# rag9704/SKIRT

Hardware: AMD Instinct MI355X
Metric: photon packets/sec (whole node), 128^3 octree, 1/2/4/8 MI355X + HBM% (higher is better)
Workload: dtype f64

## Files before the change

skirt_amd/csrc/device/engine.hip:

```cpp
#include <hip/hip_runtime.h>

#include <algorithm>
#include <cfloat>
#include <cmath>
#include <cstring>
#include <string>
#include <type_traits>
#include <vector>

#include "vor_terms.hpp"
#include "cyl2d_walk.hpp"
#include "sph_walk.hpp"
#include "geom_sample.hpp"
#include "../../../include/skirt_mcrt.h"
#include "philox.hpp"

using skirt_dev::PacketRng;

namespace {

constexpr double kDblMax = 1.7976931348623157e308;
constexpr int kBlock = 256;
constexpr int kSegWords = 3 * (kBlock / 64) * 4 / 8;
#ifndef SKIRT_LABS_BUF
// ... 55 lines not shown

struct PathRec {
    double s0, ds, tau0, dtau;
    int m, pad;
};
constexpr int kPathCap = 2048;
constexpr int kContSlots = 1 << 15;
enum ErrorBits : unsigned { ERR_TAU = 1u, ERR_PATH_CAP = 2u, ERR_QUEUE = 4u, ERR_GEOM = 8u };
static_assert(GEOMS_SHELL == SKIRT_GEOM_SHELL && GEOMS_GAMMA == SKIRT_GEOM_GAMMA && GEOMS_GAUSSIAN == SKIRT_GEOM_GAUSSIAN &&
                  GEOMS_TTAURIDISK == SKIRT_GEOM_TTAURIDISK && GEOMS_TORUS == SKIRT_GEOM_TORUS &&
                  GEOMS_CONICALSHELL == SKIRT_GEOM_CONICALSHELL,
              "geom_sample.hpp follows the kinds of skirt_mcrt.h");
template <int GRID>
constexpr bool kEnterInEvent = GRID == SKIRT_GRID_VORONOI;
constexpr int kCellIndexGroup = 2;
constexpr int kNoCell = -2;
constexpr int kOutsideShift = 28;
constexpr int kCellMaskOut = (1 << kOutsideShift) - 1;
template <int GRID>
constexpr int kSegsPerStep = GRID == SKIRT_GRID_VORONOI ? 2 : 1;

struct __attribute__((aligned(16))) DetRec {
    double Lp;
    double tau;
    int l;
    unsigned flags;
};
static_assert(sizeof(DetRec) == 24 || sizeof(DetRec) == 32, "detection record layout");
__device__ __forceinline__ unsigned rayMode(unsigned f) { return f & 3u; }
__device__ __forceinline__ unsigned rayCat(unsigned f) { return (f >> 2) & 3u; }
__device__ __forceinline__ int rayInstr(unsigned f) { return (int)((f >> 4) & 63u); }
__device__ __forceinline__ int rayLevel(unsigned f) { return (int)((f >> 10) & 255u); }
__device__ __forceinline__ int rayEll(unsigned f) { return (int)(f >> 18); }

struct LeafEntry;

struct alignas(16) BlockSite {
    double x, y, z;
    int id, pad;
};
static_assert(sizeof(BlockSite) == 32, "block site layout");

struct alignas(16) VorEntry {
    float ox, oy, oz;
    int next;
};
constexpr int kVorHead = 3;

__device__ __forceinline__ VorEntry vorEntry(const VorEntry* B, int q) {
    const float* P = reinterpret_cast<const float*>(B + kVorHead + (q & ~1));
    const int h = q & 1;
    return VorEntry{P[h], P[2 + h], P[4 + h], __float_as_int(P[6 + h])};
}

template <int N>
__device__ __forceinline__ void vorEntries(const VorEntry* B, int q0, VorEntry (&e)[N]) {
#pragma unroll
    for (int p = 0; p < N / 2; p++) {
        const float4 x = *reinterpret_cast<const float4*>(B + kVorHead + q0 + 2 * p);
        const int4 y = *reinterpret_cast<const int4*>(B + kVorHead + q0 + 2 * p + 1);
        e[2 * p] = VorEntry{x.x, x.z, __int_as_float(y.x), y.z};
        e[2 * p + 1] = VorEntry{x.y, x.w, __int_as_float(y.y), y.w};
    }
}
constexpr double kCarryTau = 0.5;
#ifndef SKIRT_POLY_EXPM1
// ... 68 lines not shown
    const double* cellCdf;
    const int* cellGuide;
    const double* cellLtot;
    double cellBias;
    const int* cellNode;
    int phase, peel;
    int ninstr;
    const DevInstr* instr;
    int nsed;
    unsigned long long npp, first, end, seed;
    unsigned long long sliceLo, sliceCnt;
    unsigned int tag;
    double minWeightReduction;
    int minScatt;
    double xi;
    int store, hasDust;
    double* labs;
    unsigned labsBytes;
    int labsGlobal;
    int labsHi;
    int labsCopies;
    unsigned labsCopyStride;
    double* tally;
    unsigned int* error;
    unsigned long long* stats;
    unsigned long long* crossed;
    int crossedBins;
    int nslots;
    double *srx, *sry, *srz, *skx, *sky, *skz, *sL, *sLth;
    int *sell, *snscatt, *sstellar, *sstate;
    int* svcell;
    uint32_t *splo, *sphi, *sblock, *sw2, *sw3, *shave;
    double *resA, *resB;
    RayRec* rays;
    DetRec* det;
    int* act[2];
    unsigned long long* claim;
    unsigned int* ctr;
    int parity, init, threshold;
    int walkBack;
    int continuous, rayCap;
    PathRec* pathBuf;
    int* pathCnt;
    int ldsMeshOff, ldsOptOff, ldsInstrOff, ldsSedOff;
    int detCopies;
};

struct __attribute__((aligned(16))) LeafEntry {
    int node;
    unsigned cl;
    double rho0;
};
constexpr int kLeafLevelShift = 27;
constexpr unsigned kLeafCellMask = (1u << kLeafLevelShift) - 1u;
constexpr int kMaxMapLevel = 9;
constexpr int kBinCellBits = 23;
constexpr unsigned kBinCellMask = (1u << kBinCellBits) - 1u;
constexpr int kMaxBinMapLevel = 7;

__host__ __device__ __forceinline__ unsigned leafBricks(int N) { return (unsigned)((N + 1) >> 1); }
__host__ __device__ __forceinline__ unsigned leafIndex(int N, unsigned x, unsigned y, unsigned z) {
    const unsigned nb = leafBricks(N);
    return ((((x >> 1) * nb + (y >> 1)) * nb + (z >> 1)) << 3) | ((x & 1u) << 2) | ((y & 1u) << 1) | (z & 1u);
}
__host__ __device__ __forceinline__ unsigned long long leafMapSize(int N) {
    const unsigned long long nb = leafBricks(N);
// ... 1012 lines not shown
            const double dx = x - sx, dy = y - sy, dz = z - sz;
            return dx * dx + dy * dy + dz * dz;
        };
        const int start = a.vorStart[m];
        double sx, sy, sz;
        siteAt(a, start, sx, sy, sz);
        const double target = d2(sx, sy, sz);
        const int cnt = reinterpret_cast<const int4*>(a.vorSlots + start + 2)->y;
        for (int q = 0; q < cnt; q++) {
            const int nxt = vorEntry(a.vorSlots + start, q).next;
            if (nxt < 0) continue;
            siteAt(a, nxt, sx, sy, sz);
            if (d2(sx, sy, sz) < target) return false;
        }
        return true;
    }
};

template <int GRID, bool ONECOMP, bool CONT, bool STORE, bool GLOBAL = false>
struct Tracer {
    const Args& a;
    const Shared& sh;
    unsigned int nseg = 0;
    unsigned int absorbs = 0, laneSlots = 0, requests = 0;
    unsigned* waveSegs;
    double* pendVal;
    unsigned* pendIdx;
    unsigned char* pendHi;
    __amdgpu_buffer_rsrc_t labsRsrc;
    unsigned copyOff = 0;
    unsigned labsOob = 0;
    int npend = 0;
    unsigned gstep = 0;

    __device__ __forceinline__ void drain() {
        static_assert(kLabsBuf >= 2 && kLabsBuf <= 64 && (kLabsBuf & (kLabsBuf - 1)) == 0, "kLabsBuf: power of 2");
        constexpr int G = 64 / kLabsBuf;
        const int lane = threadIdx.x & 63;
        const int wbase = threadIdx.x - lane;
        const int j = lane & (kLabsBuf - 1);
#pragma unroll
        for (int i = 0; i < kLabsBuf; i++) issue(i);
        npend = 0;
    }

    __device__ __forceinline__ void issue(int i) {
        constexpr int G = 64 / kLabsBuf;
        const int lane = threadIdx.x & 63;
        const int wbase = threadIdx.x - lane;
        const int j = lane & (kLabsBuf - 1);
        const int src = G * i + lane / kLabsBuf;
        const int n = __shfl(npend, src);
        const int q = j * kBlock + wbase + src;
        const unsigned idx = pendIdx[q];
        const size_t eidx = a.labsHi ? ((size_t)pendHi[q] << 32 | idx) : (size_t)idx;
        const unsigned line = (unsigned)(reinterpret_cast<size_t>(a.labs + eidx) >> 6);
        const unsigned prev = __shfl(line, lane - 1);
        const unsigned long long starts = __ballot(j < n && (j == 0 || prev != line));
        absorbs += (unsigned)__popcll(__ballot(j < n));
        requests += (unsigned)__popcll(starts);
        if constexpr (GLOBAL) {
            if (j < n) atomicAddF64(a.labs + eidx, pendVal[q]);
        } else {
            const double v = j < n ? pendVal[q] : 0.0;
            bufferAtomicAddF64(v, labsRsrc, (int)(j < n ? idx * 8u + copyOff : labsOob), 0, 0);
        }
// ... 48 lines not shown
                if (ONECOMP) albedo = sh.alb[r.ell];
                else {
                    double ksca = 0.0, kext = 0.0;
                    for (int h = 0; h < a.ncomp; h++) {
                        ksca += rho(m, h) * sh.ksca[h * a.nlambda + r.ell];
                        kext += rho(m, h) * sh.kext[h * a.nlambda + r.ell];
                    }
                    albedo = (kext > 0.0) ? ksca / kext : 0.0;
                    r.f2 += albedo * Lintm;
                }
#ifdef SKIRT_DEBUG_FILL
                printf("E S %d %.17g %.17g %.17g\n", m, ds, dtau, (1.0 - albedo) * Lintm);
#endif
                if (STORE && a.store) {
                    pendVal[npend * kBlock + threadIdx.x] = (1.0 - albedo) * Lintm;
                    if (a.labsHi) {
                        const unsigned long long e = (unsigned long long)r.ell * (unsigned)a.labsStride + (unsigned)m;
                        pendIdx[npend * kBlock + threadIdx.x] = (unsigned)e;
                        pendHi[npend * kBlock + threadIdx.x] = (unsigned char)(e >> 32);
                    } else {
                        pendIdx[npend * kBlock + threadIdx.x] = (unsigned)r.ell * (unsigned)a.labsStride + (unsigned)m;
                    }
                    npend++;
                }
            }
        } else if (r.mode == RAY_WALK) {
            if (r.tau > r.param) return false;
            r.f1 = r.tau;
            r.f2 = r.s;
        }
        return true;
    }

    __device__ __forceinline__ void load(Ray& r, unsigned id) {
        const double2* c = reinterpret_cast<const double2*>(a.rays + id);
        const double2 c0 = c[0], c1 = c[1], c2 = c[2], c3 = c[3];
        const int4 c6 = reinterpret_cast<const int4*>(c)[4];
        r.id = id;
        r.x = c0.x; r.y = c0.y; r.z = c1.x;
        r.dx = c1.y; r.dy = c2.x; r.dz = c2.y;
        r.ix = (fabs(r.dx) > 1e-15) ? 1.0 / r.dx : 0.0;
        r.iy = (fabs(r.dy) > 1e-15) ? 1.0 / r.dy : 0.0;
        r.iz = (fabs(r.dz) > 1e-15) ? 1.0 / r.dz : 0.0;
        r.param = c3.y;
        r.idx = c6.x;
        r.flags = (unsigned)c6.y;
        r.mode = rayMode(r.flags);
        r.ell = rayEll(r.flags);
        r.tau = 0;
        if (CONT && r.mode == RAY_FILL) a.pathCnt[r.idx] = 0;
#ifdef SKIRT_DEBUG_FILL
        if (r.mode == RAY_FILL)
            printf("E L %d %.17g %.17g %.17g %.17g %.17g %.17g %.17g\n", r.ell, r.x, r.y, r.z, r.dx, r.dy, r.dz, r.param);
#endif
        r.s = c3.x;
        r.kext = sh.kext[r.ell];
        r.f1 = (r.mode == RAY_FILL) ? 1.0 : 0.0;
        r.f2 = (r.mode == RAY_WALK) ? c3.x : 0.0;
        nseg = kEnterInEvent<GRID> ? ((unsigned)c6.z >> kOutsideShift) : 0u;
        if (kEnterInEvent<GRID>) {
            r.ci = c6.z & kCellMaskOut;
            r.cj = c6.w;
            r.ck = 0;
        } else if (r.mode != RAY_NONE &&
            !Grid<GRID>::begin(a, sh, r, [&](int m, double rho0, double ds) { return segment(r, m, rho0, ds); })) {
            finish(r);
            r.mode = RAY_NONE;
        }
    }

    __device__ __forceinline__ void finish(const Ray& r) {
        atomicAdd(&waveSegs[(threadIdx.x >> 6) * 3 + (r.mode == RAY_FILL ? 0 : r.mode == RAY_WALK ? 1 : 2)], nseg);
        if (a.crossed && r.mode != RAY_WALK) crossedAdd(a, nseg);
        if (r.mode == RAY_PEEL) {
            a.det[r.idx].tau = r.tau;
        } else if (r.mode == RAY_FILL) {
            a.resA[r.idx] = r.tau;
            if (!ONECOMP) a.resB[r.idx] = r.f2;
        } else {
            const double tauint = r.param;
            double s = 0;
            if (tauint > 0) {
                if (r.tau > tauint) s = r.f2 + ((tauint - r.f1) / (r.tau - r.f1)) * (r.s - r.f2);
                else s = r.f2;
            }
            a.resA[r.idx] = s;
        }
    }
};

__device__ __forceinline__ bool detectSlot(const DevInstr& ins, unsigned flags, int slot, double Lp, double Lextf,
                                           double& v) {
    v = Lextf;
    if (ins.kind != SKIRT_INSTR_FULL) return slot == 0;
    switch (rayCat(flags)) {
    case CAT_STAR_DIRECT:
        if (slot == 0) v = Lp;
        return slot <= 1;
    case CAT_STAR_SCATTERED: {
        const int lev = rayLevel(flags);
        return slot == 2 || (lev >= 1 && lev <= ins.levels && slot == 5 + lev - 1);
    }
    case CAT_DUST_DIRECT: return slot == 3;
    default: return slot == 4;
    }
}

__device__ __forceinline__ double* frameAt(const Args& a, const DevInstr& ins, int ell, int l, int slot) {
    return a.tally + ins.frameBase + ((long long)ell * ins.nx * ins.ny + l) * ins.slotStride + slot;
}

__device__ __forceinline__ void detectPeel(const Args& a, const DevInstr& ins, unsigned flags, int l, double Lp,
                                           double tau, double* sed) {
    const double Lextf = Lp * exp(-tau);
    const int nl = a.nlambda;
    const int ell = rayEll(flags);
    for (int slot = 0; slot < ins.nslots; slot++) {
        double v;
        if (!detectSlot(ins, flags, slot, Lp, Lextf, v)) continue;
        if (ins.kind != SKIRT_INSTR_FRAME) {
// ... 244 lines not shown
}

template <int GRID, bool ONECOMP, bool CONT, bool STORE, bool GLOBAL = false>
__device__ __forceinline__ void traceBody(const Args& a) {
    extern __shared__ __attribute__((aligned(16))) double lds[];
    if (blockIdx.x == 0 && threadIdx.x == 0) {
        CTR(a.ctr, 1 - a.parity) = 0;
        CTR(a.ctr, 2 + a.parity) = 0;
        CTR(a.ctr, 8 + (1 - a.parity)) = 0;
    }
    const unsigned int nfront = CTR(a.ctr, a.parity);
    if (nfront + CTR(a.ctr, 8 + a.parity) == 0) return;
    if ((unsigned long long)nfront + CTR(a.ctr, 8 + a.parity) > (unsigned long long)a.rayCap) {
        if (blockIdx.x == 0 && threadIdx.x == 0) atomicOr(a.error, ERR_QUEUE);
        return;
    }
    Shared sh = stageTables(a, lds, gridParts<GRID>() | STAGE_OPTICS);

    Tracer<GRID, ONECOMP, CONT, STORE, GLOBAL> T{a, sh};
    T.labsOob = a.labsCopies > 1 ? (unsigned)a.labsCopies * a.labsCopyStride : a.labsBytes;
    T.labsRsrc = __builtin_amdgcn_make_buffer_rsrc(a.labs, 0, (int)T.labsOob, 0x00020000);
    if (a.labsCopies > 1)
        T.copyOff = (unsigned)((blockIdx.x * (kBlock / 64) + (threadIdx.x >> 6)) % (unsigned)a.labsCopies) * a.labsCopyStride;
    T.waveSegs = reinterpret_cast<unsigned*>(lds + a.ldsInstrOff);
    T.pendVal = lds + a.ldsInstrOff + kSegWords;
    T.pendIdx = reinterpret_cast<unsigned*>(T.pendVal + kLabsBuf * kBlock);
    T.pendHi = reinterpret_cast<unsigned char*>(T.pendIdx + kLabsBuf * kBlock);
    if (threadIdx.x < 3 * (kBlock / 64)) T.waveSegs[threadIdx.x] = 0;
    __syncthreads();
    const int lane = threadIdx.x & 63;
    const unsigned int nrays = nfront + CTR(a.ctr, 8 + a.parity);
    Ray r;
    r.mode = RAY_NONE;
    bool done = false;
    constexpr unsigned kPullChunk = GRID == SKIRT_GRID_VORONOI ? 64 : 128;
    unsigned cur = 0, curEnd = 0, nxt = 0;
    bool haveNext = false;
    auto reserve = [&]() {
        unsigned int base = 0;
        if (lane == 0) base = atomicAdd(CTRP(a.ctr, 4), kPullChunk);
        return __shfl(base, 0);
    };
    while (true) {
        const bool idle = (r.mode == RAY_NONE) && !done;
        const unsigned long long imask = __ballot(idle);
        const unsigned long long amask = __ballot(r.mode != RAY_NONE);
        if (imask == 0 && amask == 0) break;
        if (imask != 0 && (amask == 0 || __popcll(imask) >= a.threshold)) {
            const unsigned int rank = (unsigned int)__popcll(imask & ((1ull << lane) - 1ull));
            const unsigned int k = (unsigned int)__popcll(imask);
            const unsigned int avail = curEnd - cur;
            if (avail < k && !haveNext) { nxt = reserve(); haveNext = true; }
            const unsigned int id = rank < avail ? cur + rank : nxt + (rank - avail);
            if (avail >= k) cur += k;
            else { cur = nxt + (k - avail); curEnd = nxt + kPullChunk; haveNext = false; }
            if (!haveNext && curEnd - cur < kPullChunk / 2 && cur < nrays) { nxt = reserve(); haveNext = true; }
            if (idle) {
                if (id >= nrays) done = true;
                else T.load(r, id < nfront ? id : (unsigned)a.rayCap - 1u - (id - nfront));
            }
            __builtin_amdgcn_s_waitcnt(0x0F70);
        }
#pragma unroll 1
        for (int it = 0; it < kStepsPerPull; it++) {
            const unsigned long long live = __ballot(r.mode != RAY_NONE);
            if (live == 0) break;
            T.laneSlots += 64;
            auto seg = [&](int m, double rho0, double ds) { return T.segment(r, m, rho0, ds); };
            if (r.mode != RAY_NONE) {
                if (!Grid<GRID>::step(a, sh, r, seg)) {
                    T.finish(r);
                    r.mode = RAY_NONE;
                }
            }
            if constexpr (!STORE) {
            } else if constexpr (kSegsPerStep<GRID> == 1) {
                T.drainStep();
            } else if (SKIRT_VOR_DRAIN2) {
                static_assert(kSegsPerStep<GRID> == 2, "two drains per step hold two adds per step");
                T.drainStep2();
            } else {
                if (__ballot(T.npend > kLabsBuf - kSegsPerStep<GRID>)) T.drain();
            }
        }
    }
    if constexpr (STORE) T.drain();
    const unsigned* ws = T.waveSegs + (threadIdx.x >> 6) * 3;
    const bool l0 = lane == 0;
    const unsigned long long vals[8] = {0, l0 ? ws[0] : 0u, l0 ? ws[1] : 0u, l0 ? ws[2] : 0u, 0,
                                        l0 ? T.absorbs : 0u, l0 ? T.laneSlots : 0u, l0 ? T.requests : 0u};
    flushStats(a, vals);
}
// ... 43 lines not shown
            }
            if (l >= 0 && ins.kind != SKIRT_INSTR_SED) atomicAddF64(frameAt(a, ins, ell, l, slot), v);
        }
        if (sub == 0) detects++;
    }
    __syncthreads();
    for (int q = threadIdx.x; copies && q < a.nsed; q += blockDim.x) {
        double v = 0.0;
        for (int g = 0; g < copies; g++) v += sh.sed[g * a.nsed + q];
        if (v != 0.0) {
            int ii = 0;
            while (ii + 1 < a.ninstr && sh.instr[ii + 1].sedOff <= q) ii++;
            atomicAddF64(a.tally + sh.instr[ii].sedBase + (q - sh.instr[ii].sedOff), v);
        }
    }
    const unsigned long long vals[8] = {0, 0, 0, 0, detects, 0, 0, 0};
    flushStats(a, vals);
}

struct Packet {
    double rx, ry, rz, kx, ky, kz, L, Lth;
    int ell, nscatt, stellar, state;
    PacketRng rng;
};

template <int GRID, bool ONECOMP>
struct Events {
    const Args& a;
    const Shared& sh;
    unsigned int packets = 0, detects = 0, segFill = 0, segWalk = 0, segPeel = 0;

    __device__ __forceinline__ double rho(int m, int h) const { return a.rho[(size_t)m * a.ncomp + h]; }

    __device__ __forceinline__ void emitRay(unsigned pos, const Packet& p, double dx, double dy, double dz, double prm,
                                            int idx, unsigned flags, int& vcell) {
        Ray r;
        r.x = p.rx; r.y = p.ry; r.z = p.rz;
        r.dx = dx; r.dy = dy; r.dz = dz;
        r.ix = (fabs(dx) > 1e-15) ? 1.0 / dx : 0.0;
        r.iy = (fabs(dy) > 1e-15) ? 1.0 / dy : 0.0;
        r.iz = (fabs(dz) > 1e-15) ? 1.0 / dz : 0.0;
        r.s = 0;
        r.ci = r.cj = 0;
        const unsigned mode = rayMode(flags);
        int4* dst = reinterpret_cast<int4*>(a.rays + pos);
        bool entered = a.hasDust;
        unsigned nseg = 0;
        if constexpr (kEnterInEvent<GRID>) {
            if (entered) entered = Grid<GRID>::beginAt(a, r, vcell, [&](int, double, double ds) {
                if (ds > 0) { r.s += ds; nseg++; }
                return true;
            });
        }
        if (kEnterInEvent<GRID> && a.crossed && mode != RAY_WALK && a.hasDust) {
            if (!entered) crossedAdd(a, 0);
        }
        if (!entered) {
            if (mode != RAY_PEEL) {
                a.resA[idx] = 0.0;
                if (!ONECOMP) a.resB[idx] = 0.0;
                if (mode == RAY_FILL && a.continuous) a.pathCnt[idx] = 0;
            }
            dst[4] = make_int4(idx, (int)RAY_NONE, 0, 0);
            return;
        }
        double2* d2 = reinterpret_cast<double2*>(dst);
        d2[0] = make_double2(r.x, r.y);
        d2[1] = make_double2(r.z, dx);
        d2[2] = make_double2(dy, dz);
        d2[3] = make_double2(r.s, prm);
        dst[4] = make_int4(idx, (int)flags, r.ci | (int)(min(nseg, 7u) << kOutsideShift), r.cj);
    }

    __device__ __forceinline__ void load(int s, Packet& p) const {
        p.rx = a.srx[s]; p.ry = a.sry[s]; p.rz = a.srz[s];
        p.kx = a.skx[s]; p.ky = a.sky[s]; p.kz = a.skz[s];
        p.L = a.sL[s]; p.Lth = a.sLth[s];
        p.ell = a.sell[s]; p.nscatt = a.snscatt[s]; p.stellar = a.sstellar[s]; p.state = a.sstate[s];
        p.rng.k0 = (uint32_t)a.seed; p.rng.k1 = (uint32_t)(a.seed >> 32); p.rng.tag = a.tag;
        p.rng.plo = a.splo[s]; p.rng.phi = a.sphi[s]; p.rng.block = a.sblock[s];
        p.rng.w2 = a.sw2[s]; p.rng.w3 = a.sw3[s]; p.rng.have = a.shave[s];
    }
    __device__ __forceinline__ void store(int s, const Packet& p) const {
        a.srx[s] = p.rx; a.sry[s] = p.ry; a.srz[s] = p.rz;
        a.skx[s] = p.kx; a.sky[s] = p.ky; a.skz[s] = p.kz;
        a.sL[s] = p.L; a.sLth[s] = p.Lth;
        a.sell[s] = p.ell; a.snscatt[s] = p.nscatt; a.sstellar[s] = p.stellar; a.sstate[s] = p.state;
        a.splo[s] = p.rng.plo; a.sphi[s] = p.rng.phi; a.sblock[s] = p.rng.block;
        a.sw2[s] = p.rng.w2; a.sw3[s] = p.rng.w3; a.shave[s] = p.rng.have;
    }

    __device__ __forceinline__ int pixel(const DevInstr& ins, const Packet& p) const {
        const double xpp = -ins.sinphi * p.rx + ins.cosphi * p.ry;
        const double ypp = -ins.cosphi * ins.costheta * p.rx - ins.sinphi * ins.costheta * p.ry + ins.sintheta * p.rz;
        const double xp = ins.cospa * xpp - ins.sinpa * ypp;
        const double yp = ins.sinpa * xpp + ins.cospa * ypp;
        const int i = static_cast<int>(floor((xp - ins.xpmin) / ins.xpsiz));
        const int j = static_cast<int>(floor((yp - ins.ypmin) / ins.ypsiz));
        return (i < 0 || i >= ins.nx || j < 0 || j >= ins.ny) ? -1 : i + ins.nx * j;
    }

    __device__ __forceinline__ bool peelWeight(const DevInstr& ins, const Packet& p, double kx, double ky, double kz,
                                               double& I) const {
        const double cosalpha = kx * ins.kobs[0] + ky * ins.kobs[1] + kz * ins.kobs[2];
// ... 276 lines not shown
        p.ell = ell;
        int h = 0;
        double L = L0;
        const int N = a.nstar;
        if (N > 1) {
            const double X = p.rng.uniform();
            const double xi = a.emissionBias;
            if (X < xi) h = max(0, min(N - 1, static_cast<int>(N * X / xi)));
            else {
                const double* Xv = a.cdf + (size_t)ell * (N + 1);
                const double q = (X - xi) / (1.0 - xi);
                if (!(q < Xv[0])) {
                    int lo = -1, hi = N;
                    while (hi - lo > 1) { const int jm = (hi + lo) >> 1; if (q < Xv[jm]) hi = jm; else lo = jm; }
                    h = lo;
                }
            }
            const double Lh = a.lum[(size_t)h * a.nlambda + ell];
            if (!(Lh > 0)) return false;
            const double Lmean = a.lumtot[ell] / N;
            L = L0 * (1.0 / (1.0 - xi + xi * Lmean / Lh));
        }
        if (!launchPosition(a.geomParam + 8 * h, a.geomTable, h, p.rng, p.rx, p.ry, p.rz)) {
            atomicOr(a.error, ERR_GEOM);
            return false;
        }
        isotropic(p.rng, p.kx, p.ky, p.kz);
        p.L = L;
        p.nscatt = 0;
        p.stellar = h;
        return true;
    }

    __device__ __forceinline__ double sampleTau(Packet& p, double taupath) const {
        double tauint = -1.0;
        if (a.xi != 0.0) {
            const double X = p.rng.uniform();
            if (X < a.xi) tauint = p.rng.uniform() * taupath;
        }
        if (tauint < 0.0) {
            if (taupath < 1e-10) tauint = p.rng.uniform() * taupath;
            else {
                const double norm = 1.0 - exp(-taupath);
                double x = -log(1.0 - p.rng.uniform() * norm);
                while (x > taupath) x = -log(1.0 - p.rng.uniform() * norm);
                tauint = x;
            }
        }
        if (a.xi != 0.0) {
            const double pr = -exp(-tauint) / expm1(-taupath);
            const double q = (1.0 - a.xi) * pr + a.xi / taupath;
            p.L = p.L * (pr / q);
        }
        return tauint;
    }
};

enum PeelKind : int { PEEL_NONE = 0, PEEL_EMISSION = 1, PEEL_SCATTER = 2 };

template <class T0, class T1>
__device__ __forceinline__ void blockReserve(T0* ctr0, T0 c0, T0& r0, T1* ctr1, T1 c1, T1& r1, unsigned long long* scratch) {
    const int lane = threadIdx.x & 63, wave = threadIdx.x >> 6;
    constexpr int W = kBlock / 64;
    T0 i0 = c0;
    T1 i1 = c1;
#pragma unroll
    for (int off = 1; off < 64; off <<= 1) {
        const T0 v0 = __shfl_up(i0, off);
        const T1 v1 = __shfl_up(i1, off);
        if (lane >= off) { i0 += v0; i1 += v1; }
    }
    if (lane == 63) { scratch[wave] = (unsigned long long)i0; scratch[W + wave] = (unsigned long long)i1; }
    __syncthreads();
    T0 w0 = 0, t0 = 0;
    T1 w1 = 0, t1 = 0;
#pragma unroll
    for (int w = 0; w < W; w++) {
        const T0 s0 = (T0)scratch[w];
        const T1 s1 = (T1)scratch[W + w];
        if (w < wave) { w0 += s0; w1 += s1; }
        t0 += s0; t1 += s1;
    }
    if (threadIdx.x == 0) scratch[2 * W] = (ctr0 && t0) ? (unsigned long long)atomicAdd(ctr0, t0) : 0ull;
    if (threadIdx.x == 64) scratch[2 * W + 1] = (ctr1 && t1) ? (unsigned long long)atomicAdd(ctr1, t1) : 0ull;
    __syncthreads();
    r0 = (T0)scratch[2 * W] + w0 + i0 - c0;
    r1 = (T1)scratch[2 * W + 1] + w1 + i1 - c1;
// ... 73 lines not shown
}

__device__ __forceinline__ unsigned long long globalPacket(const Args& a, unsigned long long j) {
    if (a.sliceCnt == a.npp) return j;
    const unsigned long long ell = j / a.sliceCnt;
    return ell * a.npp + a.sliceLo + (j - ell * a.sliceCnt);
}

template <int GRID, bool ONECOMP>
__global__ void __launch_bounds__(kBlock) SKIRT_EVENT_ATTR eventKernel(const Args a) {
    __shared__ unsigned long long resv[4 * (kBlock / 64) + 4];
    extern __shared__ __attribute__((aligned(16))) double lds[];
    if (blockIdx.x == 0 && threadIdx.x == 0) CTR(a.ctr, 4) = 0;
    if (!a.init && CTR(a.ctr, 2 + a.parity) == 0) return;
    Shared sh = stageTables(a, lds, gridParts<GRID>() | STAGE_OPTICS | STAGE_INSTR);
    Events<GRID, ONECOMP> E{a, sh};
    const int lane = threadIdx.x & 63;
    const unsigned long long total = a.end - a.first;
    const unsigned int nwork = a.init ? (unsigned)a.nslots : CTR(a.ctr, 2 + a.parity);
    const int* actIn = a.act[a.parity];
    int* actOut = a.act[1 - a.parity];
    const unsigned int stride = gridDim.x * blockDim.x;
    const unsigned int rounds = (nwork + stride - 1) / stride;
    const unsigned int w0 = blockIdx.x * blockDim.x + threadIdx.x;
    int slotNext = (w0 < nwork) ? (a.init ? (int)w0 : actIn[w0]) : 0;
    for (unsigned int round = 0; round < rounds; round++) {
        const unsigned int w = round * stride + w0;
        const bool valid = w < nwork;
        const int slot = slotNext;
        const unsigned int wn = w + stride;
        if (round + 1 < rounds) slotNext = (wn < nwork) ? (a.init ? (int)wn : actIn[wn]) : 0;
        Packet p;
        p.state = S_NEW;
        double resA = 0.0, resB = 0.0;
        int vcell = kNoCell;
        if (valid && !a.init) {
            E.load(slot, p);
            resA = a.resA[slot];
            if (!ONECOMP) resB = a.resB[slot];
            if (kEnterInEvent<GRID>) vcell = a.svcell[slot];
        }
        int peel = PEEL_NONE;
        unsigned mainMode = RAY_NONE;
        double mainParam = 0;
        double ox = 0, oy = 0, oz = 0;
        if (valid && !a.init) {
            if (p.state == S_FILL) {
                const double taupath = resA;
                if (taupath < 0.0 || isnan(taupath) || isinf(taupath)) {
                    atomicOr(a.error, ERR_TAU);
                    p.state = S_NEW;
                } else {
                    if (ONECOMP) p.L = p.L * sh.alb[p.ell] * (-expm1(-taupath));
                    else p.L = resB;
                    if (p.L <= 0 || (p.L <= p.Lth && p.nscatt >= a.minScatt)) {
                        p.state = S_NEW;
                    } else {
                        p.state = S_WALK;
                        double tauint = 0.0;
                        if (taupath != 0.0) tauint = E.sampleTau(p, taupath);
                        if (tauint > 0) { mainMode = RAY_WALK; mainParam = tauint; }
                        else resA = 0.0;
                    }
                }
            }
            if (p.state == S_WALK && mainMode == RAY_NONE) {
                const double s = resA;
                vcell = kNoCell;
                p.rx = p.rx + s * p.kx;
                p.ry = p.ry + s * p.ky;
                p.rz = p.rz + s * p.kz;
                bool ok = a.ninstr > 0 && a.peel && !a.continuous;
                if (ok && !ONECOMP) { double I; ok = E.peelWeight(sh.instr[0], p, p.kx, p.ky, p.kz, I); }
                if (ok) { peel = PEEL_SCATTER; ox = p.kx; oy = p.ky; oz = p.kz; }
                E.scatter(p);
                mainMode = RAY_FILL;
                mainParam = p.L;
                p.state = S_FILL;
            }
        }
        bool need = valid && p.state == S_NEW && mainMode == RAY_NONE;
        while (__syncthreads_or(need)) {
            unsigned long long idx = 0;
            unsigned int unused = 0;
            blockReserve<unsigned long long, unsigned int>(a.claim, need ? 1ull : 0ull, idx, nullptr, 0u, unused, resv);
            if (need) {
                if (idx >= total) need = false;
                else if (E.launch(p, globalPacket(a, a.first + idx))) {
                    vcell = kNoCell;
                    if (!(p.L > 0) && !a.crossed) {
                    } else if (a.hasDust) {
                        peel = (a.ninstr > 0 && a.peel) ? PEEL_EMISSION : PEEL_NONE;
                        mainMode = RAY_FILL;
                        mainParam = p.L;
                        p.state = S_FILL;
                        need = false;
// ... 6 lines not shown
                        }
                    }
                }
            }
        }
        int nray = 0;
        if (peel != PEEL_NONE) {
            for (int i = 0; i < a.ninstr; i++) {
                const DevInstr& ins = sh.instr[i];
                if (ins.kind == SKIRT_INSTR_FRAME && E.pixel(ins, p) < 0) continue;
                nray++;
            }
        }
        if (mainMode != RAY_NONE) nray++;
        const bool active = mainMode != RAY_NONE;
        const int npeel = nray - (mainMode != RAY_NONE ? 1 : 0);
        const bool back = a.walkBack && mainMode == RAY_WALK;
        unsigned int pos, apos, dpos, wpos;
        {
            unsigned* const ctrs[4] = {CTRP(a.ctr, a.parity), CTRP(a.ctr, 2 + (1 - a.parity)), CTRP(a.ctr, 5 + a.parity),
                                       CTRP(a.ctr, 8 + a.parity)};
            const unsigned cnt[4] = {(unsigned)nray - (back ? 1u : 0u), active ? 1u : 0u, (unsigned)npeel, back ? 1u : 0u};
            unsigned res[4];
            blockReserve4(ctrs, cnt, res, resv);
            pos = res[0]; apos = res[1]; dpos = res[2]; wpos = res[3];
        }
        if ((unsigned long long)pos + (unsigned)(nray - (back ? 1 : 0)) > (unsigned long long)a.rayCap ||
            (back && wpos >= (unsigned)a.rayCap) ||
            (unsigned long long)dpos + (unsigned)npeel > (unsigned long long)(a.rayCap - a.nslots)) {
            atomicOr(a.error, ERR_QUEUE);
            nray = 0;
        }
        int inext = 0;
        for (int k = 0; k < nray; k++) {
            double dx, dy, dz, prm;
            int idx;
            unsigned flags, at;
            if (k < npeel) {
                int i = inext, l;
                while (true) {
                    const DevInstr& ins = sh.instr[i];
                    l = ins.kind == SKIRT_INSTR_SED ? -1 : E.pixel(ins, p);
                    if (ins.kind == SKIRT_INSTR_FRAME && l < 0) { i++; continue; }
                    break;
                }
                inext = i + 1;
                const DevInstr& ins = sh.instr[i];
                double Lp = p.L;
                unsigned cat, level = 0;
                if (peel == PEEL_EMISSION) {
                    cat = p.stellar >= 0 ? CAT_STAR_DIRECT : CAT_DUST_DIRECT;
                } else {
                    double I = 0;
                    E.peelWeight(ins, p, ox, oy, oz, I);
                    Lp = p.L * I;
                    cat = p.stellar >= 0 ? CAT_STAR_SCATTERED : CAT_DUST_SCATTERED;
                    level = (unsigned)min(p.nscatt, 255);
                }
                dx = ins.kobs[0]; dy = ins.kobs[1]; dz = ins.kobs[2];
                prm = Lp;
                flags = RAY_PEEL | (cat << 2) | ((unsigned)i << 4) | (level << 10) | ((unsigned)p.ell << 18);
                idx = (int)(dpos + k);
                a.det[idx] = DetRec{Lp, 0.0, l, flags};
                at = pos++;
            } else {
                dx = p.kx; dy = p.ky; dz = p.kz;
                prm = mainParam;
                idx = slot;
                flags = mainMode | ((unsigned)p.ell << 18);
                at = back ? (unsigned)a.rayCap - 1u - wpos : pos++;
            }
            E.emitRay(at, p, dx, dy, dz, prm, idx, flags, vcell);
        }
        if (active) actOut[apos] = slot;
        if (valid) E.store(slot, p);
        if (kEnterInEvent<GRID> && valid) a.svcell[slot] = vcell;
    }
    const unsigned long long vals[8] = {E.packets, E.segFill, E.segWalk, E.segPeel, E.detects, 0, 0, 0};
    flushStats(a, vals);
}

template <int GRID, bool ONECOMP>
__global__ void __launch_bounds__(kBlock) contKernel(const Args a) {
    __shared__ unsigned long long resv[3 * (kBlock / 64) + 3];
    extern __shared__ __attribute__((aligned(16))) double lds[];
    const unsigned int nwork = CTR(a.ctr, 2 + a.parity);
    if (nwork == 0) return;
    Shared sh = stageTables(a, lds, gridParts<GRID>() | STAGE_OPTICS | STAGE_INSTR);
    Events<GRID, ONECOMP> E{a, sh};
    const int* actIn = a.act[a.parity];
    const unsigned int stride = gridDim.x * blockDim.x;
    const unsigned int rounds = (nwork + stride - 1) / stride;
    const int Nl = a.nlambda;
    for (unsigned int round = 0; round < rounds; round++) {
        const unsigned int w = round * stride + blockIdx.x * blockDim.x + threadIdx.x;
        const int slot = w < nwork ? actIn[w] : 0;
        Packet p;
        p.state = S_NEW;
        if (w < nwork) E.load(slot, p);
        const bool fill = w < nwork && p.state == S_FILL;
        const int nrec = fill ? a.pathCnt[slot] : 0;
        const PathRec* rec = a.pathBuf + (size_t)slot * kPathCap;
        auto weights = [&](int m, double* wv, double& albedo) {
            double ksca = 0.0, kext = 0.0;
            for (int h = 0; h < a.ncomp; h++) {
                const double rho = a.rho[(size_t)m * a.ncomp + h];
                wv[h] = rho * sh.ksca[h * Nl + p.ell];
                ksca += rho * sh.ksca[h * Nl + p.ell];
                kext += rho * sh.kext[h * Nl + p.ell];
// ... 107 lines not shown
    int* dCellGuide = nullptr;
    size_t cellGuideCount = 0;
    double cellBias = 0.5;
    int* dCellNode = nullptr;
    double* dLabsDust = nullptr;
    bool ownLabsDust = true;
    double* dLabsRep = nullptr;
    size_t labsRepBytes = 0;
    bool labsRepDirty = false;
    int emisNtemp = 0;
    double *dEmisVolume = nullptr, *dEmisKabs = nullptr, *dEmisSigma = nullptr, *dEmisMu = nullptr, *dEmisTv = nullptr,
           *dEmisPlanck = nullptr, *dEmisLambda = nullptr, *dEmisDlambda = nullptr, *dEmisScratch = nullptr;
    int* dDevCell = nullptr;
    std::vector<DevInstr> instr;
    DevInstr* dInstr = nullptr;
    size_t nInstrTally = 0;
    int nsed = 0;
    double *dLabs = nullptr, *dTally = nullptr;
    bool ownLabs = true, ownTally = true;
    unsigned long long *dClaim = nullptr, *dStats = nullptr;
    unsigned long long* dCrossed = nullptr;
    int crossedBins = 0;
    unsigned int *dError = nullptr, *dCtr = nullptr, *hCtr = nullptr;
    hipStream_t sD = nullptr;
    hipEvent_t evDetT = nullptr, evDet[2] = {}, evDetJoin = nullptr;
    std::vector<hipEvent_t> pollEv;
    int nslots = 0, rayCap = 0;
    bool poolPath = false;
    bool poolDetPair = false;
    void* dPool = nullptr;
    size_t poolBytes = 0;
    int traceGrid = 0, threshold = 0, slotsWanted = 0;
    int walkBack = getenv("SKIRT_AMD_WALK_BACK") ? atoi(getenv("SKIRT_AMD_WALK_BACK")) : -1;
    int traceBlocksPerCU = 0;
    int lastDetCopies = 0;
    double lastMs = 0;
    bool phaseTimed = false;
    std::vector<hipEvent_t> traceEv;
    int traceLaunches = 0;
    uint64_t packagesTotal = 0;
    double traceMs = 0;
    uint64_t traceLaunchesTotal = 0;
    int numCUs = 0;
    size_t ldsMax = 64 * 1024;
    int lastIterations = 0;
    SkirtReduceTallyFn reduce = nullptr;
    void* reduceUser = nullptr;
    bool instrReduced = false;
};

namespace {

int fail(SkirtMcrt* c, int code, const std::string& msg) {
    if (c) c->err = msg;
    return code;
}

#define HIPCHECK(ctx, call)                                                                    \
    do {                                                                                       \
        hipError_t e_ = (call);                                                                \
        if (e_ != hipSuccess) return fail(ctx, SKIRT_ERR_HIP, std::string(#call) + ": " + hipGetErrorString(e_)); \
    } while (0)

template <class T>
int upload(SkirtMcrt* c, T*& dst, const T* src, size_t n) {
    if (dst) { (void)hipFree(dst); dst = nullptr; }
// ... 45 lines not shown
int walkKind(const SkirtMcrt* c, bool hasDust) {
    if (c->gridKind < 0) return kOctreeNodes;
    if (c->gridKind != SKIRT_GRID_OCTREE) return c->gridKind;
    if (c->search == SKIRT_TREE_BOOKKEEPING) return kOctreeBookkeeping;
    if (c->mapL >= 0 && hasDust) return c->binTree ? kBinTreeMap : SKIRT_GRID_OCTREE;
    return kOctreeNodes;
}

const void* traceKernelOf(int kind, bool one, bool continuous, bool global, bool noStore) {
    return withWalk(kind, [&](auto g) {
        constexpr int G = decltype(g)::value;
        if constexpr (G != SKIRT_GRID_VORONOI)
            if (noStore) return (const void*)traceKernelNoStore<G>;
        return withBool(global, [&](auto gl) {
            constexpr bool L = decltype(gl)::value;
            if constexpr (G == SKIRT_GRID_VORONOI) {
                if (!continuous) return one ? (const void*)traceKernelVor<true, false, L> : (const void*)traceKernelVor<false, false, L>;
                return one ? (const void*)traceKernelVor<true, true, L> : (const void*)traceKernelVor<false, true, L>;
            } else {
                if (!continuous) return one ? (const void*)traceKernel<G, true, false, L> : (const void*)traceKernel<G, false, false, L>;
                return one ? (const void*)traceKernel<G, true, true, L> : (const void*)traceKernel<G, false, true, L>;
            }
        });
    });
}

int ensurePool(SkirtMcrt* c, int nslots, bool continuous, bool detPair) {
    const int ninstr = (int)c->instr.size();
    const size_t rays = (size_t)nslots * (1 + ninstr) + (continuous ? (size_t)nslots * kPathCap * ninstr : 0);
    if (rays >= (size_t)INT32_MAX) return fail(c, SKIRT_ERR_UNSUPPORTED, "ray queue too large");
    const int rayCap = (int)rays;
    const size_t path = continuous ? (size_t)nslots * (kPathCap * sizeof(PathRec) + sizeof(int)) : 0;
    const size_t bytes = (size_t)rayCap * sizeof(RayRec) + (detPair ? 2 : 1) * (size_t)(rayCap - nslots) * sizeof(DetRec) +
                         (size_t)nslots * (10 * 8 + 5 * 4 + 6 * 4 + 2 * 4) + path + 4096;
    if (c->dPool && c->nslots == nslots && c->rayCap == rayCap && c->poolPath == (path > 0) && c->poolDetPair == detPair)
        return SKIRT_OK;
    c->poolPath = path > 0;
    c->poolDetPair = detPair;
    if (c->dPool) { (void)hipFree(c->dPool); c->dPool = nullptr; }
    HIPCHECK(c, hipMalloc(&c->dPool, bytes));
    c->poolBytes = bytes;
    c->nslots = nslots;
    c->rayCap = rayCap;
    return SKIRT_OK;
}

void carvePool(SkirtMcrt* c, Args& a) {
    char* p = static_cast<char*>(c->dPool);
    const size_t n = (size_t)c->nslots;
    auto takeD = [&](double*& d) { d = reinterpret_cast<double*>(p); p += n * 8; };
    auto takeI = [&](int*& d) { d = reinterpret_cast<int*>(p); p += n * 4; };
    auto takeU = [&](uint32_t*& d) { d = reinterpret_cast<uint32_t*>(p); p += n * 4; };
    a.rays = reinterpret_cast<RayRec*>(p);
    p += (size_t)c->rayCap * sizeof(RayRec);
    a.det = reinterpret_cast<DetRec*>(p);
    p += (c->poolDetPair ? 2 : 1) * (size_t)(c->rayCap - c->nslots) * sizeof(DetRec);
    takeD(a.srx); takeD(a.sry); takeD(a.srz); takeD(a.skx); takeD(a.sky); takeD(a.skz); takeD(a.sL); takeD(a.sLth);
    takeD(a.resA); takeD(a.resB);
    takeI(a.sell); takeI(a.snscatt); takeI(a.sstellar); takeI(a.sstate); takeI(a.svcell);
    takeU(a.splo); takeU(a.sphi); takeU(a.sblock); takeU(a.sw2); takeU(a.sw3); takeU(a.shave);
    takeI(a.act[0]); takeI(a.act[1]);
    a.pathBuf = nullptr;
    a.pathCnt = nullptr;
    if (c->poolPath) {
        p = reinterpret_cast<char*>(((uintptr_t)p + 15) & ~(uintptr_t)15);
        a.pathBuf = reinterpret_cast<PathRec*>(p);
        p += n * kPathCap * sizeof(PathRec);
        takeI(a.pathCnt);
    }
    a.nslots = c->nslots;
    a.rayCap = c->rayCap;
    a.ctr = c->dCtr;
}

int planLeafMap(SkirtMcrt* c, const SkirtGridDesc* g) {
    c->mapL = -1;
    c->mapReady = false;
    if (c->dLeafMap) { (void)hipFree(c->dLeafMap); c->dLeafMap = nullptr; }
    const char* env = getenv("SKIRT_AMD_LEAFMAP");
    if (env && env[0] == '0') return SKIRT_OK;
    const bool bin = g->split_dir != nullptr;
    if (c->ndev >= (int)(1u << (bin ? kBinCellBits : kLeafLevelShift))) return SKIRT_OK;
    const int maxL = bin ? kMaxBinMapLevel : kMaxMapLevel;
    struct Item { int node, lv[3], idx[3]; };
    std::vector<Item> stack{{0, {0, 0, 0}, {0, 0, 0}}};
    std::vector<Item> nodes;
    nodes.reserve(g->nnodes);
    int L = 0;
    while (!stack.empty()) {
        const Item it = stack.back();
        stack.pop_back();
// ... 1096 lines not shown
    Args& a = pl.a;
    gridArgs(c, a);
    const int kind = pl.kind = walkKind(c, p->has_dust);
    if (kind == SKIRT_GRID_OCTREE || kind == kBinTreeMap) {
        if ((rc = ensureLeafMap(c))) return rc;
        a.leafMap = c->dLeafMap; a.treeT = c->dTreeT; a.mapL = c->mapL; a.mapN = c->mapN;
        a.mapInvX = c->mapInv[0]; a.mapInvY = c->mapInv[1]; a.mapInvZ = c->mapInv[2];
        a.mapX0 = c->mapOrigin[0]; a.mapY0 = c->mapOrigin[1]; a.mapZ0 = c->mapOrigin[2];
    }
    a.optics = c->dOptics;
    a.nstar = c->nstar; a.geomParam = c->dGeomParam; a.geomTable = c->dGeomTable; a.lum = c->dLum;
    a.lumtot = c->dLumtot; a.cdf = c->dCdf; a.emissionBias = c->emissionBias;
    a.ninstr = (int)c->instr.size(); a.instr = c->dInstr; a.nsed = c->nsed;
    a.npp = npp; a.first = first; a.end = first + count; a.seed = seed;
    a.sliceLo = sliceLo; a.sliceCnt = sliceCnt;
    a.tag = (unsigned)phase | (cycle << 2);
    a.phase = phase;
    a.peel = phase != SKIRT_PHASE_DUST_SELFABS;
    a.continuous = continuous ? 1 : 0;
    a.cellLv = c->dCellLv; a.cellCdf = c->dCellCdf; a.cellGuide = c->dCellGuide; a.cellLtot = c->dCellLtot; a.cellBias = c->cellBias;
    a.cellNode = c->dCellNode;
    a.minWeightReduction = p->min_weight_reduction; a.minScatt = p->min_scatt_events; a.xi = p->scatt_bias;
    a.store = phase == SKIRT_PHASE_STELLAR ? (p->store_absorption ? 1 : 0) : (phase == SKIRT_PHASE_DUST_SELFABS ? 1 : 0);
    a.hasDust = p->has_dust ? 1 : 0;
    if (a.store && !c->dLabs) return fail(c, SKIRT_ERR_STATE, "no Labs buffer");
    if ((rc = planLabs(c, phase, pl))) return rc;
    a.tally = c->dTally;
    a.error = c->dError; a.stats = c->dStats;
    a.crossed = c->dCrossed; a.crossedBins = c->crossedBins;
    a.claim = c->dClaim;
    a.threshold = c->threshold > 0 ? c->threshold : (c->gridKind == SKIRT_GRID_VORONOI ? 8 : 16);
    a.walkBack = c->walkBack >= 0 ? c->walkBack : (c->gridKind == SKIRT_GRID_VORONOI ? 1 : 0);
    if ((rc = planLds(c, pl))) return rc;
    c->lastWalk = walkOf(kind).stat;
    pl.traceFn = traceKernelOf(kind, a.ncomp == 1, continuous, a.labsGlobal != 0, pl.noStore);
    if (pl.ldsTrace > 64 * 1024)
        HIPCHECK(c, hipFuncSetAttribute(pl.traceFn, hipFuncAttributeMaxDynamicSharedMemorySize, (int)pl.ldsTrace));
    pl.tgrid = c->traceGrid;
    if (pl.tgrid <= 0) {
        int per = 0;
        if (hipOccupancyMaxActiveBlocksPerMultiprocessor(&per, pl.traceFn, kBlock, pl.ldsTrace) != hipSuccess || per < 1) per = 2;
        pl.tgrid = std::max(1, c->numCUs) * per;
        c->traceBlocksPerCU = per;
    }
#ifndef SKIRT_EVENT_BPC
#define SKIRT_EVENT_BPC 3
#endif
    const int ebpc = SKIRT_EVENT_BPC;
    pl.egrid = std::max(1, std::min((slots + kBlock - 1) / kBlock, std::max(1, c->numCUs) * ebpc));
    pl.dgrid = std::max(1, std::max(1, c->numCUs) * 4);
    return SKIRT_OK;
}

static int runIterations(SkirtMcrt* c, const PhasePlan& pl) {
    const int kind = pl.kind;
    const bool one = pl.a.ncomp == 1;
    auto launchEvent = [&](const Args& aa, hipStream_t st) {
        withWalk(kind, [&](auto g) {
            withBool(one, [&](auto o) {
                hipLaunchKernelGGL((eventKernel<decltype(g)::value, decltype(o)::value>), dim3(pl.egrid), dim3(kBlock),
                                   pl.ldsEvent, st, aa);
            });
        });
    };
    auto launchCont = [&](const Args& aa, hipStream_t st) {
        withWalk(kind, [&](auto g) {
// ... 437 lines not shown
```

Before: 237.9 million.

## Fuse fill-ray tau sampling and walk ray into the trace kernel

When a fill ray finishes in the trace kernel, the change samples the interaction optical depth in place using random draws precomputed by the event kernel, then relaunches the same ray as a walk ray within that trace pass. The goal is to avoid a separate event round and ray emission just to trace the walk, which saves a kernel round-trip and ray-record traffic. In exchange it adds per-slot buffers, more state in the ray records and Ray registers, and a fallback path when the rejection loop would need extra draws. The fused path is on by default except for Voronoi grids, continuous mode, and no-store octree-node walks.

```diff
diff --git a/skirt_amd/csrc/device/engine.hip b/skirt_amd/csrc/device/engine.hip
--- a/skirt_amd/csrc/device/engine.hip
+++ b/skirt_amd/csrc/device/engine.hip
@@ -111,6 +111,46 @@
 __device__ __forceinline__ int rayInstr(unsigned f) { return (int)((f >> 4) & 63u); }
 __device__ __forceinline__ int rayLevel(unsigned f) { return (int)((f >> 10) & 255u); }
 __device__ __forceinline__ int rayEll(unsigned f) { return (int)(f >> 18); }
+
+enum FillStatus : int { FILL_TERMINATED = 0, FILL_NO_WALK = 1, FILL_WALK = 2, FILL_FALLBACK = 3 };
+__device__ __forceinline__ double fillBiasWeight(double L, double tauint, double taupath, double xi) {
+    const double pr = -exp(-tauint) / expm1(-taupath);
+    const double q = (1.0 - xi) * pr + xi / taupath;
+    return L * (pr / q);
+}
+template <bool ONECOMP, class Draws>
+__device__ __forceinline__ int decideFill(double taupath, double& L, double Lsca, double albedo, double thr, double xi,
+                                          Draws& draws, double& tauint) {
+    tauint = 0.0;
+    if (taupath < 0.0 || isnan(taupath) || isinf(taupath)) return FILL_FALLBACK;
+    if (ONECOMP) L = L * albedo * (-expm1(-taupath));
+    else L = Lsca;
+    if (L <= 0 || L <= thr) return FILL_TERMINATED;
+    if (taupath == 0.0) return FILL_NO_WALK;
+    const bool biased = xi != 0.0 && draws.biased(xi);
+    const double u = draws.uniform();
+    double t;
+    if (biased || taupath < 1e-10) t = u * taupath;
+    else {
+        const double norm = 1.0 - exp(-taupath);
+        t = -log(1.0 - u * norm);
+        if (t > taupath) return FILL_FALLBACK;
+    }
+    if (xi != 0.0) L = fillBiasWeight(L, t, taupath, xi);
+    tauint = t;
+    return t > 0 ? FILL_WALK : FILL_NO_WALK;
+}
+struct FillDrawsStream {
+    PacketRng& rng;
+    __device__ __forceinline__ bool biased(double xi) { return rng.uniform() < xi; }
+    __device__ __forceinline__ double uniform() { return rng.uniform(); }
+};
+struct FillDrawsAhead {
+    bool b;
+    double u;
+    __device__ __forceinline__ bool biased(double) const { return b; }
+    __device__ __forceinline__ double uniform() const { return u; }
+};
 
 struct LeafEntry;
 
@@ -245,6 +285,9 @@
     int* svcell;
     uint32_t *splo, *sphi, *sblock, *sw2, *sw3, *shave;
     double *resA, *resB;
+    double* resS;
+    double *fuseU, *fuseThr;
+    int fuse;
     RayRec* rays;
     DetRec* det;
     int* act[2];
@@ -1323,6 +1366,11 @@
     unsigned labsOob = 0;
     int npend = 0;
     unsigned gstep = 0;
+    double fu = 0, fthr = 0;
+    static constexpr unsigned kLaneWalkOn = 1u << 31;
+    static constexpr bool kFuse = !CONT && (STORE || GRID != kOctreeNodes);
+    __device__ __forceinline__ double& fillThr(Ray& r) { return ONECOMP ? r.f2 : fthr; }
+    __device__ __forceinline__ double& fillU(Ray& r) { return (ONECOMP && !STORE) ? r.f1 : fu; }
 
     __device__ __forceinline__ void drain() {
         static_assert(kLabsBuf >= 2 && kLabsBuf <= 64 && (kLabsBuf & (kLabsBuf - 1)) == 0, "kLabsBuf: power of 2");
@@ -1437,7 +1485,7 @@
         return true;
     }
 
-    __device__ __forceinline__ void load(Ray& r, unsigned id) {
+    __device__ __forceinline__ void load(Ray& r, unsigned id, bool walkOn) {
         const double2* c = reinterpret_cast<const double2*>(a.rays + id);
         const double2 c0 = c[0], c1 = c[1], c2 = c[2], c3 = c[3];
         const int4 c6 = reinterpret_cast<const int4*>(c)[4];
@@ -1450,6 +1498,10 @@
         r.param = c3.y;
         r.idx = c6.x;
         r.flags = (unsigned)c6.y;
+        if (kFuse && walkOn) {
+            r.param = fillU(r);
+            r.flags = (r.flags & ~3u) | RAY_WALK;
+        }
         r.mode = rayMode(r.flags);
         r.ell = rayEll(r.flags);
         r.tau = 0;
@@ -1458,10 +1510,14 @@
         if (r.mode == RAY_FILL)
             printf("E L %d %.17g %.17g %.17g %.17g %.17g %.17g %.17g\n", r.ell, r.x, r.y, r.z, r.dx, r.dy, r.dz, r.param);
 #endif
-        r.s = c3.x;
+        r.s = kEnterInEvent<GRID> ? c3.x : 0.0;
         r.kext = sh.kext[r.ell];
         r.f1 = (r.mode == RAY_FILL) ? 1.0 : 0.0;
-        r.f2 = (r.mode == RAY_WALK) ? c3.x : 0.0;
+        r.f2 = (r.mode == RAY_WALK) ? r.s : 0.0;
+        if (kFuse && a.fuse && r.mode == RAY_FILL) {
+            fillU(r) = kEnterInEvent<GRID> ? a.fuseU[r.idx] : __hiloint2double(c6.w, c6.z);
+            fillThr(r) = kEnterInEvent<GRID> ? a.fuseThr[r.idx] : c3.x;
+        }
         nseg = kEnterInEvent<GRID> ? ((unsigned)c6.z >> kOutsideShift) : 0u;
         if (kEnterInEvent<GRID>) {
             r.ci = c6.z & kCellMaskOut;
@@ -1474,14 +1530,30 @@
         }
     }
 
-    __device__ __forceinline__ void finish(const Ray& r) {
+    __device__ __forceinline__ void finish(Ray& r) {
         atomicAdd(&waveSegs[(threadIdx.x >> 6) * 3 + (r.mode == RAY_FILL ? 0 : r.mode == RAY_WALK ? 1 : 2)], nseg);
         if (a.crossed && r.mode != RAY_WALK) crossedAdd(a, nseg);
+        unsigned walkOn = 0;
+        double* const walked = (kFuse && a.fuse) ? a.resS : a.resA;
         if (r.mode == RAY_PEEL) {
             a.det[r.idx].tau = r.tau;
         } else if (r.mode == RAY_FILL) {
             a.resA[r.idx] = r.tau;
             if (!ONECOMP) a.resB[r.idx] = r.f2;
+            if (kFuse && a.fuse) {
+                const double u = fillU(r);
+                FillDrawsAhead draws{u < 0.0, fabs(u)};
+                double L = r.param, tauint;
+                int st = decideFill<ONECOMP>(r.tau, L, r.f2, ONECOMP ? sh.alb[r.ell] : 0.0,
+                                              ONECOMP ? r.f2 : fthr, a.xi, draws, tauint);
+                if (a.fuse == 2 && (r.idx & 1)) st = FILL_FALLBACK;
+                if (st == FILL_WALK) {
+                    fillU(r) = tauint;
+                    walkOn = kLaneWalkOn | r.id;
+                } else {
+                    a.resS[r.idx] = -1.0;
+                }
+            }
         } else {
             const double tauint = r.param;
             double s = 0;
@@ -1489,8 +1561,9 @@
                 if (r.tau > tauint) s = r.f2 + ((tauint - r.f1) / (r.tau - r.f1)) * (r.s - r.f2);
                 else s = r.f2;
             }
-            a.resA[r.idx] = s;
-        }
+            walked[r.idx] = s;
+        }
+        r.id = walkOn;
     }
 };
 
@@ -1801,6 +1874,7 @@
     const unsigned int nrays = nfront + CTR(a.ctr, 8 + a.parity);
     Ray r;
     r.mode = RAY_NONE;
+    r.id = 0;
     bool done = false;
     constexpr unsigned kPullChunk = GRID == SKIRT_GRID_VORONOI ? 64 : 128;
     unsigned cur = 0, curEnd = 0, nxt = 0;
@@ -1816,8 +1890,10 @@
         const unsigned long long amask = __ballot(r.mode != RAY_NONE);
         if (imask == 0 && amask == 0) break;
         if (imask != 0 && (amask == 0 || __popcll(imask) >= a.threshold)) {
-            const unsigned int rank = (unsigned int)__popcll(imask & ((1ull << lane) - 1ull));
-            const unsigned int k = (unsigned int)__popcll(imask);
+            const bool walkOn = idle && (r.id & T.kLaneWalkOn) != 0;
+            const unsigned long long pmask = imask & ~__ballot(walkOn);
+            const unsigned int rank = (unsigned int)__popcll(pmask & ((1ull << lane) - 1ull));
+            const unsigned int k = (unsigned int)__popcll(pmask);
             const unsigned int avail = curEnd - cur;
             if (avail < k && !haveNext) { nxt = reserve(); haveNext = true; }
             const unsigned int id = rank < avail ? cur + rank : nxt + (rank - avail);
@@ -1825,8 +1901,8 @@
             else { cur = nxt + (k - avail); curEnd = nxt + kPullChunk; haveNext = false; }
             if (!haveNext && curEnd - cur < kPullChunk / 2 && cur < nrays) { nxt = reserve(); haveNext = true; }
             if (idle) {
-                if (id >= nrays) done = true;
-                else T.load(r, id < nfront ? id : (unsigned)a.rayCap - 1u - (id - nfront));
+                if (!walkOn && id >= nrays) done = true;
+                else T.load(r, walkOn ? r.id & ~T.kLaneWalkOn : id < nfront ? id : (unsigned)a.rayCap - 1u - (id - nfront), walkOn);
             }
             __builtin_amdgcn_s_waitcnt(0x0F70);
         }
@@ -1936,7 +2012,7 @@
 
     __device__ __forceinline__ double rho(int m, int h) const { return a.rho[(size_t)m * a.ncomp + h]; }
 
-    __device__ __forceinline__ void emitRay(unsigned pos, const Packet& p, double dx, double dy, double dz, double prm,
+    __device__ __forceinline__ bool emitRay(unsigned pos, const Packet& p, double dx, double dy, double dz, double prm,
                                             int idx, unsigned flags, int& vcell) {
         Ray r;
         r.x = p.rx; r.y = p.ry; r.z = p.rz;
@@ -1962,11 +2038,12 @@
         if (!entered) {
             if (mode != RAY_PEEL) {
                 a.resA[idx] = 0.0;
+                if (mode == RAY_WALK && a.fuse) a.resS[idx] = 0.0;
                 if (!ONECOMP) a.resB[idx] = 0.0;
                 if (mode == RAY_FILL && a.continuous) a.pathCnt[idx] = 0;
             }
             dst[4] = make_int4(idx, (int)RAY_NONE, 0, 0);
-            return;
+            return false;
         }
         double2* d2 = reinterpret_cast<double2*>(dst);
         d2[0] = make_double2(r.x, r.y);
@@ -1974,6 +2051,7 @@
         d2[2] = make_double2(dy, dz);
         d2[3] = make_double2(r.s, prm);
         dst[4] = make_int4(idx, (int)flags, r.ci | (int)(min(nseg, 7u) << kOutsideShift), r.cj);
+        return true;
     }
 
     __device__ __forceinline__ void load(int s, Packet& p) const {
@@ -2316,27 +2394,14 @@
         return true;
     }
 
-    __device__ __forceinline__ double sampleTau(Packet& p, double taupath) const {
-        double tauint = -1.0;
-        if (a.xi != 0.0) {
-            const double X = p.rng.uniform();
-            if (X < a.xi) tauint = p.rng.uniform() * taupath;
-        }
-        if (tauint < 0.0) {
-            if (taupath < 1e-10) tauint = p.rng.uniform() * taupath;
-            else {
-                const double norm = 1.0 - exp(-taupath);
-                double x = -log(1.0 - p.rng.uniform() * norm);
-                while (x > taupath) x = -log(1.0 - p.rng.uniform() * norm);
-                tauint = x;
-            }
-        }
-        if (a.xi != 0.0) {
-            const double pr = -exp(-tauint) / expm1(-taupath);
-            const double q = (1.0 - a.xi) * pr + a.xi / taupath;
-            p.L = p.L * (pr / q);
-        }
-        return tauint;
+    __device__ __forceinline__ double fillThreshold(const Packet& p) const { return p.nscatt >= a.minScatt ? p.Lth : 0.0; }
+
+    __device__ __forceinline__ double exponCutoffAgain(Packet& p, double taupath) const {
+        const double norm = 1.0 - exp(-taupath);
+        double x = -log(1.0 - p.rng.uniform() * norm);
+        while (x > taupath) x = -log(1.0 - p.rng.uniform() * norm);
+        if (a.xi != 0.0) p.L = fillBiasWeight(p.L, x, taupath, a.xi);
+        return x;
     }
 };
 
@@ -2476,12 +2541,16 @@
         if (round + 1 < rounds) slotNext = (wn < nwork) ? (a.init ? (int)wn : actIn[wn]) : 0;
         Packet p;
         p.state = S_NEW;
-        double resA = 0.0, resB = 0.0;
+        double resA = 0.0, resB = 0.0, resS = -1.0;
         int vcell = kNoCell;
         if (valid && !a.init) {
             E.load(slot, p);
             resA = a.resA[slot];
             if (!ONECOMP) resB = a.resB[slot];
+            if (a.fuse) {
+                resS = a.resS[slot];
+                if (p.state == S_WALK) resA = resS;
+            }
             if (kEnterInEvent<GRID>) vcell = a.svcell[slot];
         }
         int peel = PEEL_NONE;
@@ -2491,21 +2560,27 @@
         if (valid && !a.init) {
             if (p.state == S_FILL) {
                 const double taupath = resA;
-                if (taupath < 0.0 || isnan(taupath) || isinf(taupath)) {
-                    atomicOr(a.error, ERR_TAU);
+                FillDrawsStream draws{p.rng};
+                double tauint;
+                int st = decideFill<ONECOMP>(taupath, p.L, resB, ONECOMP ? sh.alb[p.ell] : 0.0, E.fillThreshold(p), a.xi,
+                                             draws, tauint);
+                if (st == FILL_FALLBACK) {
+                    if (taupath < 0.0 || isnan(taupath) || isinf(taupath)) {
+                        atomicOr(a.error, ERR_TAU);
+                        st = FILL_TERMINATED;
+                    } else {
+                        tauint = E.exponCutoffAgain(p, taupath);
+                        st = tauint > 0 ? FILL_WALK : FILL_NO_WALK;
+                    }
+                    resS = -1.0;
+                }
+                if (st == FILL_TERMINATED) {
                     p.state = S_NEW;
                 } else {
-                    if (ONECOMP) p.L = p.L * sh.alb[p.ell] * (-expm1(-taupath));
-                    else p.L = resB;
-                    if (p.L <= 0 || (p.L <= p.Lth && p.nscatt >= a.minScatt)) {
-                        p.state = S_NEW;
-                    } else {
-                        p.state = S_WALK;
-                        double tauint = 0.0;
-                        if (taupath != 0.0) tauint = E.sampleTau(p, taupath);
-                        if (tauint > 0) { mainMode = RAY_WALK; mainParam = tauint; }
-                        else resA = 0.0;
-                    }
+                    p.state = S_WALK;
+                    if (st == FILL_WALK && resS >= 0.0) resA = resS;
+                    else if (st == FILL_WALK) { mainMode = RAY_WALK; mainParam = tauint; }
+                    else resA = 0.0;
                 }
             }
             if (p.state == S_WALK && mainMode == RAY_NONE) {
@@ -2578,6 +2653,7 @@
             nray = 0;
         }
         int inext = 0;
+        int fillAt = -1;
         for (int k = 0; k < nray; k++) {
             double dx, dy, dz, prm;
             int idx;
@@ -2616,11 +2692,27 @@
                 flags = mainMode | ((unsigned)p.ell << 18);
                 at = back ? (unsigned)a.rayCap - 1u - wpos : pos++;
             }
-            E.emitRay(at, p, dx, dy, dz, prm, idx, flags, vcell);
+            const bool in = E.emitRay(at, p, dx, dy, dz, prm, idx, flags, vcell);
+            if (k >= npeel && in && mainMode == RAY_FILL) fillAt = (int)at;
         }
         if (active) actOut[apos] = slot;
         if (valid) E.store(slot, p);
         if (kEnterInEvent<GRID> && valid) a.svcell[slot] = vcell;
+        if (a.fuse && fillAt >= 0) {
+            PacketRng ahead = p.rng;
+            const bool biased = a.xi != 0.0 && ahead.uniform() < a.xi;
+            const double u = ahead.uniform();
+            const double fu = biased ? -u : u, fthr = E.fillThreshold(p);
+            RayRec* rec = a.rays + fillAt;
+            if (kEnterInEvent<GRID>) {
+                a.fuseU[slot] = fu;
+                a.fuseThr[slot] = fthr;
+            } else {
+                rec->s0 = fthr;
+                rec->ci = __double2loint(fu);
+                rec->cj = __double2hiint(fu);
+            }
+        }
     }
     const unsigned long long vals[8] = {E.packets, E.segFill, E.segWalk, E.segPeel, E.detects, 0, 0, 0};
     flushStats(a, vals);
@@ -2794,6 +2886,7 @@
     size_t poolBytes = 0;
     int traceGrid = 0, threshold = 0, slotsWanted = 0;
     int walkBack = getenv("SKIRT_AMD_WALK_BACK") ? atoi(getenv("SKIRT_AMD_WALK_BACK")) : -1;
+    int fuseWalk = getenv("SKIRT_AMD_FUSE_WALK") ? atoi(getenv("SKIRT_AMD_FUSE_WALK")) : -1;
     int traceBlocksPerCU = 0;
     int lastDetCopies = 0;
     double lastMs = 0;
@@ -2905,7 +2998,7 @@
     const int rayCap = (int)rays;
     const size_t path = continuous ? (size_t)nslots * (kPathCap * sizeof(PathRec) + sizeof(int)) : 0;
     const size_t bytes = (size_t)rayCap * sizeof(RayRec) + (detPair ? 2 : 1) * (size_t)(rayCap - nslots) * sizeof(DetRec) +
-                         (size_t)nslots * (10 * 8 + 5 * 4 + 6 * 4 + 2 * 4) + path + 4096;
+                         (size_t)nslots * (13 * 8 + 5 * 4 + 6 * 4 + 2 * 4) + path + 4096;
     if (c->dPool && c->nslots == nslots && c->rayCap == rayCap && c->poolPath == (path > 0) && c->poolDetPair == detPair)
         return SKIRT_OK;
     c->poolPath = path > 0;
@@ -2929,7 +3022,7 @@
     a.det = reinterpret_cast<DetRec*>(p);
     p += (c->poolDetPair ? 2 : 1) * (size_t)(c->rayCap - c->nslots) * sizeof(DetRec);
     takeD(a.srx); takeD(a.sry); takeD(a.srz); takeD(a.skx); takeD(a.sky); takeD(a.skz); takeD(a.sL); takeD(a.sLth);
-    takeD(a.resA); takeD(a.resB);
+    takeD(a.resA); takeD(a.resB); takeD(a.resS); takeD(a.fuseU); takeD(a.fuseThr);
     takeI(a.sell); takeI(a.snscatt); takeI(a.sstellar); takeI(a.sstate); takeI(a.svcell);
     takeU(a.splo); takeU(a.sphi); takeU(a.sblock); takeU(a.sw2); takeU(a.sw3); takeU(a.shave);
     takeI(a.act[0]); takeI(a.act[1]);
@@ -4092,6 +4185,9 @@
     a.threshold = c->threshold > 0 ? c->threshold : (c->gridKind == SKIRT_GRID_VORONOI ? 8 : 16);
     a.walkBack = c->walkBack >= 0 ? c->walkBack : (c->gridKind == SKIRT_GRID_VORONOI ? 1 : 0);
     if ((rc = planLds(c, pl))) return rc;
+    a.fuse = (continuous || (pl.noStore && kind == kOctreeNodes)) ? 0
+             : c->fuseWalk >= 0                                    ? std::min(c->fuseWalk, 2)
+                                                                   : (c->gridKind == SKIRT_GRID_VORONOI ? 0 : 1);
     c->lastWalk = walkOf(kind).stat;
     pl.traceFn = traceKernelOf(kind, a.ncomp == 1, continuous, a.labsGlobal != 0, pl.noStore);
     if (pl.ldsTrace > 64 * 1024)
```

Measured after the change: 245.4 million (median of 6 runs). 3.2% higher.
